# adrientremblay/Skillshot_Learning

Hardware: NVIDIA B200
Metric: env_steps_per_sec (higher is better)
Workload: dtype f64

## Files before the change

skillshot_learning_b200/csrc/ss_env.cu:

```cuda
#include <cuda_runtime.h>
#include <stdint.h>
#include <stdlib.h>

#include "../../include/skillshot_b200.h"
#include "ss_env_core.cuh"
#include "ss_env_pp.cuh"
#include "ss_launch.cuh"

namespace {

using namespace ss;

constexpr int kBlock = 64;
constexpr int kRowF4 = 7;

struct StatePlanes {
    double2 *rot;
    double2 *qrot;
    int4 *ia;
    int4 *ib;
};
__host__ __device__ inline StatePlanes planes_of(void *state, int64_t n) {
    char *b = (char *)state;
    return StatePlanes{(double2 *)b, (double2 *)(b + 16 * n), (int4 *)(b + 32 * n), (int4 *)(b + 48 * n)};
}

__device__ __forceinline__ void load_env(const StatePlanes &s, int64_t i, Env &e) {
    double2 r = s.rot[i], q = s.qrot[i];
    int4 a = s.ia[i], b = s.ib[i];
    unpack(e, r.x, r.y, q.x, q.y, Int4{a.x, a.y, a.z, a.w}, Int4{b.x, b.y, b.z, b.w});
}
__device__ __forceinline__ void store_env(const StatePlanes &s, int64_t i, const Env &e) {
    Int4 a, b;
    pack(e, a, b);
    s.rot[i] = make_double2(e.prot[0], e.prot[1]);
    s.qrot[i] = make_double2(e.qrot[0], e.qrot[1]);
    s.ia[i] = make_int4(a.x, a.y, a.z, a.w);
    s.ib[i] = make_int4(b.x, b.y, b.z, b.w);
}
__device__ __forceinline__ Speeds load_speeds(const void *speeds, int64_t n, int64_t i) {
    const char *b = (const char *)speeds;
    double2 a = ((const double2 *)b)[i];
    const double *p1 = (const double *)(b + 16 * n) + 2 * i;
    long long cm = ((const long long *)(b + 16 * n))[2 * i + 1];
    return Speeds{a.x, a.y, p1[0], (int)cm, 1.0f / (float)cm};
}

struct SmemSink {
    float4 *row;
    __device__ __forceinline__ void put(int j, float a, float b, float c, float d) { row[j] = make_float4(a, b, c, d); }
};

__device__ __noinline__ void count_episode(unsigned long long *stats, int len, int winner, int tick_limit) {
    const int width = tick_limit > 0 ? (tick_limit + 63) / 64 : 32;
    atomicAdd(stats + 0, 1ull);
    atomicAdd(stats + (winner == 1 ? 1 : winner == 2 ? 2 : 3), 1ull);
    atomicAdd(stats + 4, (unsigned long long)len);
    atomicAdd(stats + 8 + min(63, len / width), 1ull);
}

struct StepArgs {
    void *state;
    int64_t n;
    const float4 *actions;
    float4 *obs_out;
    float2 *reward_out;
    uint8_t *done_out;
    uint8_t *winner_out;
    float4 *obs_out2;
    uint16_t *done_rows_out;
    const void *speeds;
    uint32_t *status;
    unsigned long long *stats;
    uint8_t *packed_out;
    TickParams P;
    int n_ticks, obs_every_tick;
};

template <bool OBS, bool CARRY, bool SPEEDS, int MINB = 1, bool STATS = false, bool PDL = false, int BLK = kBlock>
__global__ void __launch_bounds__(BLK, MINB) step_kernel(const StepArgs A) {
    __shared__ float4 tile[OBS ? BLK / 32 : 1][OBS ? 32 * kRowF4 : 1];
    const int lane = threadIdx.x & 31, warp = threadIdx.x >> 5;
    const int64_t i = (int64_t)blockIdx.x * BLK + threadIdx.x;
    const int64_t warp_base = i - lane;
    const bool active = i < A.n;
    const StatePlanes S = planes_of(A.state, A.n);

    if (PDL) asm volatile("griddepcontrol.wait;" ::: "memory");
    Env e;
    Speeds k = default_speeds();
    if (active) {
        load_env(S, i, e);
        if (SPEEDS) k = load_speeds(A.speeds, A.n, i);
    } else {
        reset_env(e, 50, 50, 200, 200);
    }
    if (PDL) asm volatile("griddepcontrol.launch_dependents;");
    uint32_t status = 0;
    const bool write_reward = A.reward_out && A.P.reward_mode != SS_REWARD_NONE;
    Trig tr;
    if (CARRY) trig_of(e, tr);

    float4 a_next = make_float4(0.f, 0.f, 0.f, 0.f);
    if (active) a_next = __ldg(A.actions + i);
    for (int t = 0; t < A.n_ticks; ++t) {
        const int64_t row = (int64_t)t * A.n + i;
        const float4 a = a_next;
        if (active && t + 1 < A.n_ticks) a_next = __ldg(A.actions + row + A.n);
        const bool want_obs = OBS && (A.obs_every_tick || t == A.n_ticks - 1);
        float r[2];
        int done, winner;
        SmemSink sink{&tile[OBS ? warp : 0][OBS ? lane * kRowF4 : 0]};
        const int ticks_before = !STATS ? 0 : (!e.live || (A.P.tick_limit > 0 && e.ticks >= A.P.tick_limit)) ? -1 : e.ticks;
        tick_env<OBS, CARRY>(e, a.x, a.y, a.z, a.w, k, A.P, (uint64_t)i, t, want_obs, status, tr, r, done, winner, sink);
        if (STATS && active && done && ticks_before >= 0)
            count_episode(A.stats, ticks_before + 1, winner, (int)A.P.tick_limit);
        if (active) {
            if (write_reward) A.reward_out[row] = make_float2(r[0], r[1]);
            if (A.done_out) A.done_out[row] = (uint8_t)done;
            if (A.done_rows_out) A.done_rows_out[row] = (uint16_t)(winner ? 0x0101 : 0);
            if (A.winner_out) A.winner_out[row] = (uint8_t)winner;
        }
        if (OBS && want_obs) {
            __syncwarp();
            const int64_t tick_off = A.obs_every_tick ? (int64_t)t * A.n * 6 : 0;
            float4 *dst = A.obs_out + tick_off + warp_base * 6;
#pragma unroll
            for (int j = 0; j < 6; ++j) {
                int idx = j * 32 + lane, rw = idx / 6, cl = idx - rw * 6;
                if (warp_base + rw < A.n) {
                    const float4 v = tile[warp][rw * kRowF4 + cl];
                    dst[idx] = v;
                    if (A.obs_out2) A.obs_out2[warp_base * 6 + idx] = v;
                }
            }
            __syncwarp();
        }
    }
    if (active) store_env(S, i, e);
    if (status && A.status) atomicOr(A.status, status);
}

constexpr int kBlockPP = 64;
constexpr double kRound = 6755399441055744.0;

__device__ __forceinline__ double coord(int x) { return __hiloint2double(0x43380000, x); }
__device__ __forceinline__ int icoord(double w) { return __double2loint(w); }
__device__ __forceinline__ double with_low(double w, int lo) { return __hiloint2double(__double2hiint(w), lo); }

struct Lane {
    double rot;
    double s3, c3;
    double qs5, qc5;
    double wx, wy, ux, uy;
    int cd, age, valid, live, winner, ticks;
};

__device__ __forceinline__ float clip_unit_nan(float v) {
    float r;
    asm("max.NaN.f32 %0, %1, 0fBF800000;" : "=f"(r) : "f"(v));
    asm("min.NaN.f32 %0, %1, 0f3F800000;" : "=f"(r) : "f"(r));
    return r;
}
__device__ __forceinline__ bool either_nan(double a, double b) {
    int p;
    asm("{ .reg .pred q; setp.nan.f64 q, %1, %2; selp.s32 %0, 1, 0, q; }" : "=r"(p) : "d"(a), "d"(b));
    return p != 0;
}

__device__ __forceinline__ void lane_reset(Lane &L, double *qrot, int x, int y) {
    L.wx = coord(x); L.wy = coord(y); L.rot = 0.0;
    L.ux = coord(0); L.uy = coord(0); *qrot = 0.0; L.cd = 0; L.age = 0; L.valid = 0;
    L.ticks = 0; L.live = 1; L.winner = 0;
    L.s3 = 0.0; L.c3 = 3.0; L.qs5 = 0.0; L.qc5 = 5.0;
}

struct LaneIo {
    uint32_t idx;
    uint32_t n2;
    const float2 *actions;
    float *reward;
    uint8_t *flags;
};

struct Turn {
    double rot, s, c;
};

template <bool CHECKED>
__device__ __forceinline__ void turn_from(Turn &out, double rot_before, float look) {
    out.rot = fma((double)clip_unit_nan(look), 0.25, rot_before);
    if (CHECKED) sincos_d(out.rot, &out.s, &out.c);
    else sincos_d_unchecked(out.rot, &out.s, &out.c);
}

enum { OUT_FLAGS = 0, OUT_TERMINAL = 1, OUT_PACKED = 2 };

template <int TERMINAL, bool CHECKED>
__device__ __forceinline__ void lane_tick(Lane &L, double *qrot, const float move, const float look_next, const Turn &now, Turn &next,
                                          const StepArgs &A, LaneIo &io, int lane, int P, int64_t env, int tick, int limit,
                                          bool write_zero, bool &nan_seen) {
    turn_from<CHECKED>(next, now.rot, look_next);
    const double speed = (double)clip_unit_nan(move);
    const double vx = sub(sub(L.wx, kRound), mul(L.s3, speed));
    const double vy = sub(sub(L.wy, kRound), mul(L.c3, speed));
    const double cx = add(vx, kRound), cy = add(vy, kRound);
    const bool ok = (unsigned)icoord(cx) <= (unsigned)(kBoard - kPlayerSize) &&
                    (unsigned)icoord(cy) <= (unsigned)(kBoard - kPlayerSize);
    L.wx = with_low(L.wx, ok ? icoord(cx) : icoord(L.wx));
    L.wy = with_low(L.wy, ok ? icoord(cy) : icoord(L.wy));
    L.rot = now.rot;
    L.s3 = mul(now.s, 3.0); L.c3 = mul(now.c, 3.0);
    if (L.cd <= 0) {
        L.ux = with_low(L.ux, icoord(L.wx)); L.uy = with_low(L.uy, icoord(L.wy));
        *qrot = now.rot;
        L.qs5 = mul(now.s, 5.0); L.qc5 = mul(now.c, 5.0);
        L.valid = 1; L.cd = 15; L.age = 0;
    }
    const int lv = L.live;
    const double zx = sub(sub(L.ux, kRound), L.qs5);
    const double zy = sub(sub(L.uy, kRound), L.qc5);
    if (either_nan(vx, zx)) nan_seen = true;
    const double dx = add(zx, kRound), dy = add(zy, kRound);
    const bool inb = (unsigned)icoord(dx) <= (unsigned)(kBoard - kProjSize) &&
                     (unsigned)icoord(dy) <= (unsigned)(kBoard - kProjSize);
    const bool fly = lv && L.valid && inb;
    L.ux = with_low(L.ux, fly ? icoord(dx) : icoord(L.ux));
    L.uy = with_low(L.uy, fly ? icoord(dy) : icoord(L.uy));
    L.valid = lv ? (int)fly : L.valid;
    L.ticks += lv; L.cd -= lv; L.age += lv;
    const uint32_t mine = (uint32_t)icoord(L.ux) | ((uint32_t)icoord(L.uy) << 8) | ((uint32_t)L.valid << 16);
    const uint32_t theirs = __shfl_xor_sync(0xffffffffu, mine, 1);
    const int jx = theirs & 255, jy = (theirs >> 8) & 255, px = icoord(L.wx), py = icoord(L.wy);
    const bool in_x = (unsigned)(jx + kProjSize - px) <= (unsigned)kPlayerSize || (unsigned)(jx - px) <= (unsigned)kPlayerSize;
    const bool in_y = (unsigned)(jy - py) <= (unsigned)kPlayerSize || (unsigned)(jy - kProjSize - py) <= (unsigned)kPlayerSize;
    const bool hit = lv && (theirs >> 16) && in_x && in_y;
    const uint32_t pair = (__ballot_sync(0xffffffffu, hit) >> (lane & 30)) & 3u;
    float r = 0.f;
    if (pair) {
        L.winner = (pair & 1u) ? 1 : 2;
        L.live = 0;
        r = (L.winner - 1 == P) ? -1.f : 1.f;
    }
    const bool done = !L.live || L.ticks >= limit;
    if (TERMINAL == OUT_PACKED) {
        if (!P) io.flags[io.idx >> 1] = (uint8_t)((int)done | (L.winner << 1) | (pair ? 8 : 0));
    } else {
        if (TERMINAL == OUT_TERMINAL) io.reward[io.idx] = r;
        else if (write_zero) io.reward[io.idx] = 0.f;
        io.flags[io.idx >> 1] = (uint8_t)(P ? L.winner : (int)done);
    }
    io.idx += io.n2;
    if (A.P.auto_reset && done) {
        int x = P ? 200 : 50, y = x;
        if (A.P.reset_mode == SS_RESET_RANDOM) {
            const uint64_t ctr = A.P.counter + (uint64_t)tick;
            const U4 u = philox4x32_10(U4{(uint32_t)env, (uint32_t)((uint64_t)env >> 32), (uint32_t)ctr, (uint32_t)(ctr >> 32)},
                                       (uint32_t)A.P.seed, (uint32_t)(A.P.seed >> 32));
            x = rand_coord(P ? u.z : u.x); y = rand_coord(P ? u.w : u.y);
        }
        lane_reset(L, qrot, x, y);
        turn_from<CHECKED>(next, 0.0, look_next);
    }
}

template <int TERMINAL, bool CHECKED>
__device__ __forceinline__ void lane_loop(Lane &L, double *qrot, const StepArgs &A, LaneIo &io, int lane, int P, int64_t env,
                                          bool &nan_seen) {
    const int limit = A.P.tick_limit > 0 ? (int)min((int64_t)0x7fffffff, A.P.tick_limit) : 0x7fffffff;
    const bool write_zero = TERMINAL == OUT_FLAGS && A.reward_out && A.P.reward_mode != SS_REWARD_NONE;
    const int T = A.n_ticks;
    const float2 zero = make_float2(0.f, 0.f);
    float2 a0 = __ldg(io.actions + io.idx);
    float2 qa = T > 1 ? __ldg(io.actions + (io.idx + io.n2)) : zero;
    float2 qb = T > 2 ? __ldg(io.actions + (io.idx + 2 * io.n2)) : zero;
    Turn ta, tb;
    turn_from<CHECKED>(ta, L.rot, a0.y);
    float move = a0.x;
    for (int t = 0; t < T; t += 2) {
        lane_tick<TERMINAL, CHECKED>(L, qrot, move, qa.y, ta, tb, A, io, lane, P, env, t, limit, write_zero, nan_seen);
        move = qa.x;
        qa = (t + 3 < T) ? __ldg(io.actions + (io.idx + 2 * io.n2)) : zero;
        if (t + 1 < T) {
            lane_tick<TERMINAL, CHECKED>(L, qrot, move, qb.y, tb, ta, A, io, lane, P, env, t + 1, limit, write_zero, nan_seen);
            move = qb.x;
            qb = (t + 4 < T) ? __ldg(io.actions + (io.idx + 2 * io.n2)) : zero;
        }
    }
}

template <int TERMINAL, int BLK = kBlockPP>
__global__ void __launch_bounds__(BLK, 896 / BLK) step_pp_kernel(const StepArgs A) {
    constexpr int kBlockPP = BLK;
    __shared__ double qrot_sh[kBlockPP];
    const int lane = threadIdx.x & 31, P = lane & 1;
    int64_t gl = (int64_t)blockIdx.x * kBlockPP + threadIdx.x;
    gl = min(gl, 2 * A.n - 2 + P);
    const int64_t env = gl >> 1;
    char *const base = (char *)A.state;
    double *const qrot = &qrot_sh[threadIdx.x];
    Lane L;
    {
        L.rot = ((const double *)base)[gl];
        *qrot = ((const double *)(base + 16 * A.n))[gl];
        const int4 a = ((const int4 *)(base + 32 * A.n))[env], b = ((const int4 *)(base + 48 * A.n))[env];
        const uint32_t pp = (uint32_t)a.x >> (16 * P), qq = (uint32_t)a.y >> (16 * P), f = (uint32_t)b.w;
        L.wx = coord(pp & 255); L.wy = coord((pp >> 8) & 255); L.ux = coord(qq & 255); L.uy = coord((qq >> 8) & 255);
        L.cd = P ? a.w : a.z; L.age = P ? b.y : b.x; L.ticks = b.z;
        L.valid = (f >> P) & 1; L.live = (f >> 2) & 1; L.winner = (f >> 4) & 3;
        double s, c;
        sincos_d(L.rot, &s, &c);
        L.s3 = mul(s, 3.0); L.c3 = mul(c, 3.0);
        sincos_d(*qrot, &s, &c);
        L.qs5 = mul(s, 5.0); L.qc5 = mul(c, 5.0);
    }
    bool nan_seen = false;
    LaneIo io;
    io.idx = (uint32_t)gl; io.n2 = (uint32_t)(2 * A.n);
    io.actions = (const float2 *)A.actions;
    io.reward = (float *)A.reward_out;
    io.flags = TERMINAL == OUT_PACKED ? A.packed_out : (P ? A.winner_out : A.done_out);
    const bool in_range = fabs(L.rot) + 0.25 * (double)A.n_ticks + 1.0 < 1.0e5;
    if (__all_sync(0xffffffffu, in_range)) lane_loop<TERMINAL, false>(L, qrot, A, io, lane, P, env, nan_seen);
    else lane_loop<TERMINAL, true>(L, qrot, A, io, lane, P, env, nan_seen);
    const int v_other = __shfl_xor_sync(0xffffffffu, L.valid, 1);
    ((double *)base)[gl] = L.rot;
    ((double *)(base + 16 * A.n))[gl] = *qrot;
    char *ia = base + 32 * A.n + env * 16, *ib = base + 48 * A.n + env * 16;
    ((uint16_t *)ia)[P] = (uint16_t)(icoord(L.wx) | (icoord(L.wy) << 8));
    ((uint16_t *)ia)[2 + P] = (uint16_t)(icoord(L.ux) | (icoord(L.uy) << 8));
    ((int *)ia)[2 + P] = L.cd;
    ((int *)ib)[P] = L.age;
    if (!P) ((int2 *)ib)[1] = make_int2(L.ticks, L.valid | (v_other << 1) | (L.live << 2) | (L.winner << 4));
    if (nan_seen && A.status) atomicOr(A.status, kStatusNaN);
}

struct SelfPlayRows {
    static constexpr bool kPool = false;
};
struct PoolRows {
    static constexpr bool kPool = true;
    int64_t S, b;
    const float2 *opp_actions;
    float4 *opp_obs;
    unsigned long long *pool_stats;
};

__device__ __noinline__ void count_pool_game(unsigned long long *c, int len, int winner, int learner_player) {
    atomicAdd(c + 0, 1ull);
    atomicAdd(c + (winner == 0 ? 3 : winner == learner_player + 1 ? 2 : 1), 1ull);
    atomicAdd(c + 4, (unsigned long long)len);
}

template <bool STATS, class Rows>
__global__ void __launch_bounds__(kBlockPP) step_pp_obs_kernel(const StepArgs A, const Rows R) {
    __shared__ float4 tile[kBlockPP / 32][96];
    const int lane = threadIdx.x & 31, warp = threadIdx.x >> 5, P = lane & 1;
    const int64_t g0 = (int64_t)blockIdx.x * kBlockPP + threadIdx.x;
    const int64_t last = 2 * A.n - 2 + P;
    const bool active = g0 <= last;
    const int64_t gl = active ? g0 : last;
    const int64_t env = gl >> 1;
    sslaunch::griddep_wait();
    sslaunch::griddep_launch();
    bool learner = true;
    int64_t row = gl, block = 0;
    int learner_player = 0;
    if constexpr (Rows::kPool) {
        if (env >= R.S) {
            const int64_t j = env - R.S;
            block = j / R.b;
            learner_player = j - block * R.b >= (R.b >> 1) ? 1 : 0;
            learner = P == learner_player;
            row = learner ? 2 * R.S + j : j;
        }
    }
    sspp::LaneState L;
    sspp::lane_load((const char *)A.state, A.n, gl, L);
    const float2 *act = (const float2 *)A.actions;
    if constexpr (Rows::kPool) {
        if (!learner) act = R.opp_actions;
    }
    const float2 a = __ldg(act + row);
    uint32_t status = 0;
    sspp::LaneTrig T;
    sspp::lane_trig(L, T);
    sspp::LaneTickOut out;
    sspp::lane_obs_tick(L, T, a.x, a.y, A.P, (uint64_t)env, A.P.counter, lane, P, status, out);
    const int v_other = __shfl_xor_sync(0xffffffffu, L.valid, 1);
    if (active) {
        sspp::lane_store((char *)A.state, A.n, gl, L, v_other);
        if (learner && A.reward_out && A.P.reward_mode != SS_REWARD_NONE) ((float *)A.reward_out)[row] = out.reward;
        uint8_t *flag = P ? A.winner_out : A.done_out;
        if (flag) flag[env] = (uint8_t)(P ? out.winner : out.done);
        if (learner && A.done_rows_out) ((uint8_t *)A.done_rows_out)[row] = out.winner ? 1 : 0;
        if (STATS && !P && out.episode_len >= 0) count_episode(A.stats, out.episode_len, out.winner, (int)A.P.tick_limit);
        if constexpr (Rows::kPool) {
            if (!P && R.pool_stats && env >= R.S && out.episode_len >= 0)
                count_pool_game(R.pool_stats + block * 8, out.episode_len, out.winner, learner_player);
        }
    }
    if constexpr (Rows::kPool) {
        const unsigned lmask = __ballot_sync(0xffffffffu, active && learner), omask = __ballot_sync(0xffffffffu, active && !learner);
        const unsigned below = (1u << lane) - 1u;
        const int nl = __popc(lmask), no = __popc(omask);
        const int64_t l0 = __shfl_sync(0xffffffffu, row, lmask ? __ffs(lmask) - 1 : 0);
        const int64_t o0 = __shfl_sync(0xffffffffu, row, omask ? __ffs(omask) - 1 : 0);
        const int slot = learner ? __popc(lmask & below) : nl + __popc(omask & below);
        if (active) {
#pragma unroll
            for (int j = 0; j < 3; ++j) tile[warp][slot * 3 + j] = out.obs[j];
        }
        __syncwarp();
#pragma unroll
        for (int j = 0; j < 3; ++j) {
            const int idx = j * 32 + lane;
            if (idx < 3 * nl) {
                const float4 v = tile[warp][idx];
                A.obs_out[l0 * 3 + idx] = v;
                if (A.obs_out2) A.obs_out2[l0 * 3 + idx] = v;
            } else if (idx < 3 * (nl + no)) {
                R.opp_obs[o0 * 3 + (idx - 3 * nl)] = tile[warp][idx];
            }
        }
    } else {
#pragma unroll
        for (int j = 0; j < 3; ++j) tile[warp][lane * 3 + j] = out.obs[j];
        __syncwarp();
        const int64_t warp_base = (g0 - lane) * 3;
        const int64_t total = 2 * A.n * 3;
#pragma unroll
        for (int j = 0; j < 3; ++j) {
            const int64_t idx = warp_base + j * 32 + lane;
            if (idx < total) {
                const float4 v = tile[warp][j * 32 + lane];
                A.obs_out[idx] = v;
                if (A.obs_out2) A.obs_out2[idx] = v;
            }
        }
    }
    if (status && A.status) atomicOr(A.status, status);
}


struct TilesArgs {
    StepArgs S;
    int *tile_ready;
    int64_t units;
    int grid_fwd;
};

template <bool STATS>
__global__ void __launch_bounds__(32, 16) step_pp_tiles_kernel(const TilesArgs T) {
    const StepArgs &A = T.S;
    const int lane = threadIdx.x, P = lane & 1;
    const int per_step = 4 * T.grid_fwd;
    const int64_t j = blockIdx.x / per_step;
    const int c = (int)(blockIdx.x % per_step) >> 2, quarter = blockIdx.x & 3;
    const int64_t u0 = T.units * c / T.grid_fwd, u1 = T.units * (c + 1) / T.grid_fwd;
    const int64_t tile = u0 + j;
    if (tile >= u1) return;
    const int64_t rows = 2 * A.n;
    uint32_t status = 0;
    if (lane == 0) {
        int seen = 0;
        uint32_t spins = 0;
        for (;;) {
            asm volatile("ld.acquire.gpu.global.s32 %0, [%1];" : "=r"(seen) : "l"(T.tile_ready + tile) : "memory");
            if (seen >= 4) break;
            if (++spins > (1u << 20)) { status |= SS_STATUS_ROLLOUT_TIMEOUT; break; }
            __nanosleep(200);
        }
    }
    __syncwarp();
    const int64_t g0 = tile * 128 + quarter * 32 + lane;
    const int64_t last = rows - 2 + P;
    const bool active = g0 <= last;
    const int64_t gl = active ? g0 : last;
    const int64_t env = gl >> 1;
    sspp::LaneState L;
    sspp::lane_load((const char *)A.state, A.n, gl, L);
    const float2 a = __ldcg((const float2 *)A.actions + gl);
    sspp::LaneTrig Tr;
    sspp::lane_trig(L, Tr);
    sspp::LaneTickOut out;
    sspp::lane_obs_tick(L, Tr, a.x, a.y, A.P, (uint64_t)env, A.P.counter, lane, P, status, out);
    const int v_other = __shfl_xor_sync(0xffffffffu, L.valid, 1);
    if (active) {
        sspp::lane_store((char *)A.state, A.n, gl, L, v_other);
        if (A.reward_out && A.P.reward_mode != SS_REWARD_NONE) ((float *)A.reward_out)[gl] = out.reward;
        uint8_t *flag = P ? A.winner_out : A.done_out;
        if (flag) flag[env] = (uint8_t)(P ? out.winner : out.done);
        if (A.done_rows_out) ((uint8_t *)A.done_rows_out)[gl] = out.winner ? 1 : 0;
        if (STATS && !P && out.episode_len >= 0) sspp::count_episode_pp(A.stats, out.episode_len, out.winner, (int)A.P.tick_limit);
#pragma unroll
        for (int q = 0; q < 3; ++q) {
            A.obs_out[gl * 3 + q] = out.obs[q];
            if (A.obs_out2) A.obs_out2[gl * 3 + q] = out.obs[q];
        }
    }
    __syncwarp();
    if (lane == 0) atomicSub(T.tile_ready + tile, 1);
    if (status && A.status) atomicOr(A.status, status);
}

__global__ void reset_kernel(void *state, int64_t n, const uint8_t *mask, int reset_mode,
                             const int32_t *positions, uint64_t seed, uint64_t counter) {
    int64_t i = (int64_t)blockIdx.x * blockDim.x + threadIdx.x;
    if (i >= n) return;
    if (mask && !mask[i]) return;
    Env e;
    if (reset_mode == SS_RESET_GIVEN) {
        const int4 p = ((const int4 *)positions)[i];
        reset_env(e, p.x, p.y, p.z, p.w);
    } else if (reset_mode == SS_RESET_RANDOM) {
        reset_random(e, seed, (uint64_t)i, counter);
    } else {
        reset_env(e, 50, 50, 200, 200);
    }
    store_env(planes_of(state, n), i, e);
}

template <bool SPEEDS>
__global__ void features_kernel(const void *state, int64_t n, double *feat_out, double *obs_out,
                                int32_t *general_out, const void *speeds) {
    int64_t i = (int64_t)blockIdx.x * blockDim.x + threadIdx.x;
    if (i >= n) return;
    Env e;
    load_env(planes_of((void *)state, n), i, e);
    Speeds k = default_speeds();
    if (SPEEDS) k = load_speeds(speeds, n, i);
    if (general_out) {
        general_out[i * 3 + 0] = e.live; general_out[i * 3 + 1] = e.ticks; general_out[i * 3 + 2] = e.winner;
    }
    if (feat_out) {
        double f[kNumFeat];
        features_of<0>(e, f);
        for (int j = 0; j < kNumFeat; ++j) feat_out[(i * 2 + 0) * kNumFeat + j] = f[j];
        features_of<1>(e, f);
        for (int j = 0; j < kNumFeat; ++j) feat_out[(i * 2 + 1) * kNumFeat + j] = f[j];
    }
    if (obs_out) {
        double o[kNumObs];
        View v0 = view_of<0, false>(e), v1 = view_of<1, false>(e);
        obs_of<0>(e, v0, k, o);
        for (int j = 0; j < kNumObs; ++j) obs_out[(i * 2 + 0) * kNumObs + j] = o[j];
        obs_of<1>(e, v1, k, o);
        for (int j = 0; j < kNumObs; ++j) obs_out[(i * 2 + 1) * kNumObs + j] = o[j];
    }
}

__global__ void export_kernel(const void *state, int64_t n, int64_t first, int64_t count,
                              int32_t *ints, double *rots) {
    int64_t j = (int64_t)blockIdx.x * blockDim.x + threadIdx.x;
    if (j >= count) return;
    Env e;
    load_env(planes_of((void *)state, n), first + j, e);
    int32_t *o = ints + j * SS_EXPORT_INTS;
    o[0] = e.px[0]; o[1] = e.px[1]; o[2] = e.py[0]; o[3] = e.py[1];
    o[4] = e.qx[0]; o[5] = e.qx[1]; o[6] = e.qy[0]; o[7] = e.qy[1];
    o[8] = e.cd[0]; o[9] = e.cd[1]; o[10] = e.age[0]; o[11] = e.age[1];
    o[12] = e.valid[0]; o[13] = e.valid[1]; o[14] = e.ticks; o[15] = e.live; o[16] = e.winner;
    double *r = rots + j * 4;
    r[0] = e.prot[0]; r[1] = e.prot[1]; r[2] = e.qrot[0]; r[3] = e.qrot[1];
}

__global__ void import_kernel(void *state, int64_t n, int64_t first, int64_t count,
                              const int32_t *ints, const double *rots) {
    int64_t j = (int64_t)blockIdx.x * blockDim.x + threadIdx.x;
    if (j >= count) return;
    Env e;
    const int32_t *o = ints + j * SS_EXPORT_INTS;
    e.px[0] = o[0] & 255; e.px[1] = o[1] & 255; e.py[0] = o[2] & 255; e.py[1] = o[3] & 255;
    e.qx[0] = o[4] & 255; e.qx[1] = o[5] & 255; e.qy[0] = o[6] & 255; e.qy[1] = o[7] & 255;
    e.cd[0] = o[8]; e.cd[1] = o[9]; e.age[0] = o[10]; e.age[1] = o[11];
    e.valid[0] = o[12] != 0; e.valid[1] = o[13] != 0; e.ticks = o[14]; e.live = o[15] != 0; e.winner = o[16] & 3;
    const double *r = rots + j * 4;
    e.prot[0] = r[0]; e.prot[1] = r[1]; e.qrot[0] = r[2]; e.qrot[1] = r[3];
    store_env(planes_of(state, n), first + j, e);
}

template <int P>
__device__ void apply_player_op(Env &e, int op, double value, const Speeds &k, uint32_t &status) {
    double s, c;
    switch (op) {
        case SS_OP_MOVE_DIRECTION_FLOAT:
            sincos_d(e.prot[P], &s, &c);
            move_direction_float<P>(e, value, s, c, k, status);
            break;
        case SS_OP_MOVE_LOOK_FLOAT: move_look_float<P>(e, value, k); break;
        case SS_OP_SHOOT: move_shoot<P>(e, k); break;
        case SS_OP_MOVE_FORWARDS:
            sincos_d(e.prot[P], &s, &c);
            move_direction_float<P>(e, 1.0, s, c, k, status);
            break;
        case SS_OP_MOVE_BACKWARDS:
            sincos_d(e.prot[P], &s, &c);
            move_direction_float<P>(e, -1.0, s, c, k, status);
            break;
        case SS_OP_LOOK_LEFT: e.prot[P] = add(e.prot[P], k.speed_look); break;
        case SS_OP_LOOK_RIGHT: e.prot[P] = sub(e.prot[P], k.speed_look); break;
        default: break;
    }
}

__global__ void apply_kernel(void *state, int64_t n, int64_t env, int player, int op, double value,
                             const void *speeds, uint32_t *status_out) {
    Env e;
    const StatePlanes S = planes_of(state, n);
    load_env(S, env, e);
    Speeds k = speeds ? load_speeds(speeds, n, env) : default_speeds();
    uint32_t status = 0;
    if (op == SS_OP_GAME_TICK) {
        if (e.live) {
            double s, c;
            e.ticks += 1;
            sincos_d(e.qrot[0], &s, &c); proj_tick<0>(e, s, c, k, status);
            sincos_d(e.qrot[1], &s, &c); proj_tick<1>(e, s, c, k, status);
            check_collision(e);
        }
    } else if (player == 0) {
        apply_player_op<0>(e, op, value, k, status);
    } else {
        apply_player_op<1>(e, op, value, k, status);
    }
    store_env(S, env, e);
    if (status && status_out) atomicOr(status_out, status);
}

struct MatchStepArgs {
    void *state;
    int64_t n, split, tick_limit;
    const float2 *actions;
// ... 432 lines not shown
```

Before: 84.90 billion.

## Compute per-tick trig in f32 with exact f64 fallback near rounding boundaries

Replaces the per-tick f64 sincos and f64 position arithmetic with an f32 sincos and integer positions. Each rounded offset is checked against a safety margin and recomputed in f64 only when it lies near a .5 boundary. Projectile steps are precomputed once per spawn as integer offsets, so most ticks avoid f64 entirely. This is meant to cut FP64 throughput cost on the hot path, in exchange for extra branching, more code and a subtle exactness argument that relies on the margins.

```diff
diff --git a/skillshot_learning_b200/csrc/ss_env.cu b/skillshot_learning_b200/csrc/ss_env.cu
--- a/skillshot_learning_b200/csrc/ss_env.cu
+++ b/skillshot_learning_b200/csrc/ss_env.cu
@@ -5,6 +5,7 @@
 #include "../../include/skillshot_b200.h"
 #include "ss_env_core.cuh"
 #include "ss_env_pp.cuh"
+#include "ss_round_f32.cuh"
 #include "ss_launch.cuh"
 
 namespace {
@@ -156,6 +157,17 @@
     int cd, age, valid, live, winner, ticks;
 };
 
+struct LaneF {
+    double rot;
+    float s, c;
+    int px, py, ux, uy;
+    int sx, sy;
+    int qexact;
+    int cd, age, valid, live, winner, ticks;
+};
+
+struct ProjShared { double rot, s5, c5; };
+
 __device__ __forceinline__ float clip_unit_nan(float v) {
     float r;
     asm("max.NaN.f32 %0, %1, 0fBF800000;" : "=f"(r) : "f"(v));
@@ -167,12 +179,20 @@
     asm("{ .reg .pred q; setp.nan.f64 q, %1, %2; selp.s32 %0, 1, 0, q; }" : "=r"(p) : "d"(a), "d"(b));
     return p != 0;
 }
+__device__ __forceinline__ double i2d_exact(int x) { return sub(coord(x), kRound); }
+__device__ __forceinline__ int round_i(double v) { return icoord(add(v, kRound)); }
 
 __device__ __forceinline__ void lane_reset(Lane &L, double *qrot, int x, int y) {
     L.wx = coord(x); L.wy = coord(y); L.rot = 0.0;
     L.ux = coord(0); L.uy = coord(0); *qrot = 0.0; L.cd = 0; L.age = 0; L.valid = 0;
     L.ticks = 0; L.live = 1; L.winner = 0;
     L.s3 = 0.0; L.c3 = 3.0; L.qs5 = 0.0; L.qc5 = 5.0;
+}
+__device__ __forceinline__ void lane_reset(LaneF &L, ProjShared *q, int x, int y) {
+    L.px = x; L.py = y; L.rot = 0.0;
+    L.ux = 0; L.uy = 0; q->rot = 0.0; L.cd = 0; L.age = 0; L.valid = 0;
+    L.ticks = 0; L.live = 1; L.winner = 0;
+    L.s = 0.f; L.c = 1.f; L.sx = 0; L.sy = -5; L.qexact = 0;
 }
 
 struct LaneIo {
@@ -186,21 +206,74 @@
 struct Turn {
     double rot, s, c;
 };
-
-template <bool CHECKED>
+struct TurnF {
+    double rot;
+    float s, c;
+};
+
+__device__ __forceinline__ double turned(double rot_before, float look) {
+    return fma((double)clip_unit_nan(look), 0.25, rot_before);
+}
 __device__ __forceinline__ void turn_from(Turn &out, double rot_before, float look) {
-    out.rot = fma((double)clip_unit_nan(look), 0.25, rot_before);
-    if (CHECKED) sincos_d(out.rot, &out.s, &out.c);
-    else sincos_d_unchecked(out.rot, &out.s, &out.c);
+    out.rot = turned(rot_before, look);
+    sincos_d(out.rot, &out.s, &out.c);
+}
+__device__ __forceinline__ void turn_from(TurnF &out, double rot_before, float look) {
+    out.rot = turned(rot_before, look);
+    sincos_f32(out.rot, &out.s, &out.c);
 }
 
 enum { OUT_FLAGS = 0, OUT_TERMINAL = 1, OUT_PACKED = 2 };
 
-template <int TERMINAL, bool CHECKED>
+struct TickCtx {
+    const StepArgs &A;
+    LaneIo &io;
+    int lane, P;
+    int64_t env;
+    int limit;
+    bool write_zero;
+};
+
+template <int TERMINAL>
+__device__ __forceinline__ bool tick_end(const TickCtx &C, int px, int py, int ux, int uy, int valid, int lv, int &live, int &winner,
+                                         int ticks, int tick, int &x, int &y) {
+    const uint32_t mine = (uint32_t)ux | ((uint32_t)uy << 8) | ((uint32_t)valid << 16);
+    const uint32_t theirs = __shfl_xor_sync(0xffffffffu, mine, 1);
+    const int jx = theirs & 255, jy = (theirs >> 8) & 255;
+    const bool in_x = (unsigned)(jx + kProjSize - px) <= (unsigned)kPlayerSize || (unsigned)(jx - px) <= (unsigned)kPlayerSize;
+    const bool in_y = (unsigned)(jy - py) <= (unsigned)kPlayerSize || (unsigned)(jy - kProjSize - py) <= (unsigned)kPlayerSize;
+    const bool hit = lv && (theirs >> 16) && in_x && in_y;
+    const uint32_t pair = (__ballot_sync(0xffffffffu, hit) >> (C.lane & 30)) & 3u;
+    float r = 0.f;
+    if (pair) {
+        winner = (pair & 1u) ? 1 : 2;
+        live = 0;
+        r = (winner - 1 == C.P) ? -1.f : 1.f;
+    }
+    const bool done = !live || ticks >= C.limit;
+    if (TERMINAL == OUT_PACKED) {
+        if (!C.P) C.io.flags[C.io.idx >> 1] = (uint8_t)((int)done | (winner << 1) | (pair ? 8 : 0));
+    } else {
+        if (TERMINAL == OUT_TERMINAL) C.io.reward[C.io.idx] = r;
+        else if (C.write_zero) C.io.reward[C.io.idx] = 0.f;
+        C.io.flags[C.io.idx >> 1] = (uint8_t)(C.P ? winner : (int)done);
+    }
+    C.io.idx += C.io.n2;
+    if (!(C.A.P.auto_reset && done)) return false;
+    x = C.P ? 200 : 50; y = x;
+    if (C.A.P.reset_mode == SS_RESET_RANDOM) {
+        const uint64_t ctr = C.A.P.counter + (uint64_t)tick;
+        const U4 u = philox4x32_10(U4{(uint32_t)C.env, (uint32_t)((uint64_t)C.env >> 32), (uint32_t)ctr, (uint32_t)(ctr >> 32)},
+                                   (uint32_t)C.A.P.seed, (uint32_t)(C.A.P.seed >> 32));
+        x = rand_coord(C.P ? u.z : u.x); y = rand_coord(C.P ? u.w : u.y);
+    }
+    return true;
+}
+
+template <int TERMINAL>
 __device__ __forceinline__ void lane_tick(Lane &L, double *qrot, const float move, const float look_next, const Turn &now, Turn &next,
-                                          const StepArgs &A, LaneIo &io, int lane, int P, int64_t env, int tick, int limit,
-                                          bool write_zero, bool &nan_seen) {
-    turn_from<CHECKED>(next, now.rot, look_next);
+                                          const TickCtx &C, int tick, bool &nan_seen) {
+    turn_from(next, now.rot, look_next);
     const double speed = (double)clip_unit_nan(move);
     const double vx = sub(sub(L.wx, kRound), mul(L.s3, speed));
     const double vy = sub(sub(L.wy, kRound), mul(L.c3, speed));
@@ -229,60 +302,81 @@
     L.uy = with_low(L.uy, fly ? icoord(dy) : icoord(L.uy));
     L.valid = lv ? (int)fly : L.valid;
     L.ticks += lv; L.cd -= lv; L.age += lv;
-    const uint32_t mine = (uint32_t)icoord(L.ux) | ((uint32_t)icoord(L.uy) << 8) | ((uint32_t)L.valid << 16);
-    const uint32_t theirs = __shfl_xor_sync(0xffffffffu, mine, 1);
-    const int jx = theirs & 255, jy = (theirs >> 8) & 255, px = icoord(L.wx), py = icoord(L.wy);
-    const bool in_x = (unsigned)(jx + kProjSize - px) <= (unsigned)kPlayerSize || (unsigned)(jx - px) <= (unsigned)kPlayerSize;
-    const bool in_y = (unsigned)(jy - py) <= (unsigned)kPlayerSize || (unsigned)(jy - kProjSize - py) <= (unsigned)kPlayerSize;
-    const bool hit = lv && (theirs >> 16) && in_x && in_y;
-    const uint32_t pair = (__ballot_sync(0xffffffffu, hit) >> (lane & 30)) & 3u;
-    float r = 0.f;
-    if (pair) {
-        L.winner = (pair & 1u) ? 1 : 2;
-        L.live = 0;
-        r = (L.winner - 1 == P) ? -1.f : 1.f;
-    }
-    const bool done = !L.live || L.ticks >= limit;
-    if (TERMINAL == OUT_PACKED) {
-        if (!P) io.flags[io.idx >> 1] = (uint8_t)((int)done | (L.winner << 1) | (pair ? 8 : 0));
+    int x, y;
+    if (tick_end<TERMINAL>(C, icoord(L.wx), icoord(L.wy), icoord(L.ux), icoord(L.uy), L.valid, lv, L.live, L.winner, L.ticks, tick,
+                           x, y)) {
+        lane_reset(L, qrot, x, y);
+        turn_from(next, 0.0, look_next);
+    }
+}
+
+__device__ __forceinline__ void spawn_step(LaneF &L, ProjShared *q, double rot, float s, float c) {
+    L.qexact = proj_step(rot, s, c, &L.sx, &L.sy, &q->s5, &q->c5) == 2;
+}
+
+template <int TERMINAL>
+__device__ __forceinline__ void lane_tick(LaneF &L, ProjShared *q, const float move, const float look_next, const TurnF &now,
+                                          TurnF &next, const TickCtx &C, int tick, bool &nan_seen) {
+    turn_from(next, now.rot, look_next);
+    const float speed = clip_unit_nan(move);
+    int nx, ny;
+    if (move_offsets_f32(L.s, L.c, speed, &nx, &ny)) {
+        nx = L.px - nx; ny = L.py - ny;
     } else {
-        if (TERMINAL == OUT_TERMINAL) io.reward[io.idx] = r;
-        else if (write_zero) io.reward[io.idx] = 0.f;
-        io.flags[io.idx >> 1] = (uint8_t)(P ? L.winner : (int)done);
-    }
-    io.idx += io.n2;
-    if (A.P.auto_reset && done) {
-        int x = P ? 200 : 50, y = x;
-        if (A.P.reset_mode == SS_RESET_RANDOM) {
-            const uint64_t ctr = A.P.counter + (uint64_t)tick;
-            const U4 u = philox4x32_10(U4{(uint32_t)env, (uint32_t)((uint64_t)env >> 32), (uint32_t)ctr, (uint32_t)(ctr >> 32)},
-                                       (uint32_t)A.P.seed, (uint32_t)(A.P.seed >> 32));
-            x = rand_coord(P ? u.z : u.x); y = rand_coord(P ? u.w : u.y);
-        }
-        lane_reset(L, qrot, x, y);
-        turn_from<CHECKED>(next, 0.0, look_next);
-    }
-}
-
-template <int TERMINAL, bool CHECKED>
-__device__ __forceinline__ void lane_loop(Lane &L, double *qrot, const StepArgs &A, LaneIo &io, int lane, int P, int64_t env,
-                                          bool &nan_seen) {
-    const int limit = A.P.tick_limit > 0 ? (int)min((int64_t)0x7fffffff, A.P.tick_limit) : 0x7fffffff;
-    const bool write_zero = TERMINAL == OUT_FLAGS && A.reward_out && A.P.reward_mode != SS_REWARD_NONE;
-    const int T = A.n_ticks;
+        double s, c;
+        sincos_d_unchecked(L.rot, &s, &c);
+        const double sp = (double)speed;
+        const double vx = sub(i2d_exact(L.px), mul(mul(s, 3.0), sp));
+        const double vy = sub(i2d_exact(L.py), mul(mul(c, 3.0), sp));
+        if (either_nan(vx, vy)) nan_seen = true;
+        nx = round_i(vx); ny = round_i(vy);
+    }
+    if ((unsigned)nx <= (unsigned)(kBoard - kPlayerSize) && (unsigned)ny <= (unsigned)(kBoard - kPlayerSize)) {
+        L.px = nx; L.py = ny;
+    }
+    L.rot = now.rot; L.s = now.s; L.c = now.c;
+    if (L.cd <= 0) {
+        L.ux = L.px; L.uy = L.py;
+        q->rot = now.rot;
+        spawn_step(L, q, now.rot, now.s, now.c);
+        L.valid = 1; L.cd = 15; L.age = 0;
+    }
+    const int lv = L.live;
+    int mx = L.ux + L.sx, my = L.uy + L.sy;
+    if (L.qexact) {
+        const double zx = sub(i2d_exact(L.ux), q->s5), zy = sub(i2d_exact(L.uy), q->c5);
+        if (either_nan(zx, zy)) nan_seen = true;
+        mx = round_i(zx); my = round_i(zy);
+    }
+    const bool inb = (unsigned)mx <= (unsigned)(kBoard - kProjSize) && (unsigned)my <= (unsigned)(kBoard - kProjSize);
+    const bool fly = lv && L.valid && inb;
+    if (fly) { L.ux = mx; L.uy = my; }
+    L.valid = lv ? (int)fly : L.valid;
+    L.ticks += lv; L.cd -= lv; L.age += lv;
+    int x, y;
+    if (tick_end<TERMINAL>(C, L.px, L.py, L.ux, L.uy, L.valid, lv, L.live, L.winner, L.ticks, tick, x, y)) {
+        lane_reset(L, q, x, y);
+        turn_from(next, 0.0, look_next);
+    }
+}
+
+template <int TERMINAL, class LaneT, class TurnT, class Q>
+__device__ __forceinline__ void lane_loop(LaneT &L, Q *q, const TickCtx &C, bool &nan_seen) {
+    LaneIo &io = C.io;
+    const int T = C.A.n_ticks;
     const float2 zero = make_float2(0.f, 0.f);
     float2 a0 = __ldg(io.actions + io.idx);
     float2 qa = T > 1 ? __ldg(io.actions + (io.idx + io.n2)) : zero;
     float2 qb = T > 2 ? __ldg(io.actions + (io.idx + 2 * io.n2)) : zero;
-    Turn ta, tb;
-    turn_from<CHECKED>(ta, L.rot, a0.y);
+    TurnT ta, tb;
+    turn_from(ta, L.rot, a0.y);
     float move = a0.x;
     for (int t = 0; t < T; t += 2) {
-        lane_tick<TERMINAL, CHECKED>(L, qrot, move, qa.y, ta, tb, A, io, lane, P, env, t, limit, write_zero, nan_seen);
+        lane_tick<TERMINAL>(L, q, move, qa.y, ta, tb, C, t, nan_seen);
         move = qa.x;
         qa = (t + 3 < T) ? __ldg(io.actions + (io.idx + 2 * io.n2)) : zero;
         if (t + 1 < T) {
-            lane_tick<TERMINAL, CHECKED>(L, qrot, move, qb.y, tb, ta, A, io, lane, P, env, t + 1, limit, write_zero, nan_seen);
+            lane_tick<TERMINAL>(L, q, move, qb.y, tb, ta, C, t + 1, nan_seen);
             move = qb.x;
             qb = (t + 4 < T) ? __ldg(io.actions + (io.idx + 2 * io.n2)) : zero;
         }
@@ -292,27 +386,22 @@
 template <int TERMINAL, int BLK = kBlockPP>
 __global__ void __launch_bounds__(BLK, 896 / BLK) step_pp_kernel(const StepArgs A) {
     constexpr int kBlockPP = BLK;
-    __shared__ double qrot_sh[kBlockPP];
+    __shared__ ProjShared proj_sh[kBlockPP];
     const int lane = threadIdx.x & 31, P = lane & 1;
     int64_t gl = (int64_t)blockIdx.x * kBlockPP + threadIdx.x;
     gl = min(gl, 2 * A.n - 2 + P);
     const int64_t env = gl >> 1;
     char *const base = (char *)A.state;
-    double *const qrot = &qrot_sh[threadIdx.x];
-    Lane L;
+    ProjShared *const q = &proj_sh[threadIdx.x];
+    LaneF L;
     {
         L.rot = ((const double *)base)[gl];
-        *qrot = ((const double *)(base + 16 * A.n))[gl];
+        q->rot = ((const double *)(base + 16 * A.n))[gl];
         const int4 a = ((const int4 *)(base + 32 * A.n))[env], b = ((const int4 *)(base + 48 * A.n))[env];
         const uint32_t pp = (uint32_t)a.x >> (16 * P), qq = (uint32_t)a.y >> (16 * P), f = (uint32_t)b.w;
-        L.wx = coord(pp & 255); L.wy = coord((pp >> 8) & 255); L.ux = coord(qq & 255); L.uy = coord((qq >> 8) & 255);
+        L.px = pp & 255; L.py = (pp >> 8) & 255; L.ux = qq & 255; L.uy = (qq >> 8) & 255;
         L.cd = P ? a.w : a.z; L.age = P ? b.y : b.x; L.ticks = b.z;
         L.valid = (f >> P) & 1; L.live = (f >> 2) & 1; L.winner = (f >> 4) & 3;
-        double s, c;
-        sincos_d(L.rot, &s, &c);
-        L.s3 = mul(s, 3.0); L.c3 = mul(c, 3.0);
-        sincos_d(*qrot, &s, &c);
-        L.qs5 = mul(s, 5.0); L.qc5 = mul(c, 5.0);
     }
     bool nan_seen = false;
     LaneIo io;
@@ -320,15 +409,34 @@
     io.actions = (const float2 *)A.actions;
     io.reward = (float *)A.reward_out;
     io.flags = TERMINAL == OUT_PACKED ? A.packed_out : (P ? A.winner_out : A.done_out);
+    const TickCtx C{A, io, lane, P, env,
+                    A.P.tick_limit > 0 ? (int)min((int64_t)0x7fffffff, A.P.tick_limit) : 0x7fffffff,
+                    TERMINAL == OUT_FLAGS && A.reward_out && A.P.reward_mode != SS_REWARD_NONE};
     const bool in_range = fabs(L.rot) + 0.25 * (double)A.n_ticks + 1.0 < 1.0e5;
-    if (__all_sync(0xffffffffu, in_range)) lane_loop<TERMINAL, false>(L, qrot, A, io, lane, P, env, nan_seen);
-    else lane_loop<TERMINAL, true>(L, qrot, A, io, lane, P, env, nan_seen);
+    double s, c;
+    sincos_d(q->rot, &s, &c);
+    if (__all_sync(0xffffffffu, in_range)) {
+        sincos_f32(L.rot, &L.s, &L.c);
+        L.qexact = !proj_step_f64(s, c, &L.sx, &L.sy);
+        if (L.qexact) { q->s5 = mul(s, 5.0); q->c5 = mul(c, 5.0); }
+        lane_loop<TERMINAL, LaneF, TurnF>(L, q, C, nan_seen);
+    } else {
+        Lane D;
+        D.rot = L.rot; D.wx = coord(L.px); D.wy = coord(L.py); D.ux = coord(L.ux); D.uy = coord(L.uy);
+        D.cd = L.cd; D.age = L.age; D.valid = L.valid; D.live = L.live; D.winner = L.winner; D.ticks = L.ticks;
+        D.qs5 = mul(s, 5.0); D.qc5 = mul(c, 5.0);
+        sincos_d(D.rot, &s, &c);
+        D.s3 = mul(s, 3.0); D.c3 = mul(c, 3.0);
+        lane_loop<TERMINAL, Lane, Turn>(D, &q->rot, C, nan_seen);
+        L.rot = D.rot; L.px = icoord(D.wx); L.py = icoord(D.wy); L.ux = icoord(D.ux); L.uy = icoord(D.uy);
+        L.cd = D.cd; L.age = D.age; L.valid = D.valid; L.live = D.live; L.winner = D.winner; L.ticks = D.ticks;
+    }
     const int v_other = __shfl_xor_sync(0xffffffffu, L.valid, 1);
     ((double *)base)[gl] = L.rot;
-    ((double *)(base + 16 * A.n))[gl] = *qrot;
+    ((double *)(base + 16 * A.n))[gl] = q->rot;
     char *ia = base + 32 * A.n + env * 16, *ib = base + 48 * A.n + env * 16;
-    ((uint16_t *)ia)[P] = (uint16_t)(icoord(L.wx) | (icoord(L.wy) << 8));
-    ((uint16_t *)ia)[2 + P] = (uint16_t)(icoord(L.ux) | (icoord(L.uy) << 8));
+    ((uint16_t *)ia)[P] = (uint16_t)(L.px | (L.py << 8));
+    ((uint16_t *)ia)[2 + P] = (uint16_t)(L.ux | (L.uy << 8));
     ((int *)ia)[2 + P] = L.cd;
     ((int *)ib)[P] = L.age;
     if (!P) ((int2 *)ib)[1] = make_int2(L.ticks, L.valid | (v_other << 1) | (L.live << 2) | (L.winner << 4));
diff --git a/skillshot_learning_b200/csrc/ss_round_f32.cuh b/skillshot_learning_b200/csrc/ss_round_f32.cuh
--- /dev/null
+++ b/skillshot_learning_b200/csrc/ss_round_f32.cuh
@@ -0,0 +1,117 @@
+#pragma once
+#include "ss_env_core.cuh"
+
+namespace ss {
+
+SS_HD float fmul_rn(float a, float b) {
+#ifdef __CUDA_ARCH__
+    return __fmul_rn(a, b);
+#else
+    return a * b;
+#endif
+}
+SS_HD float fadd_rn(float a, float b) {
+#ifdef __CUDA_ARCH__
+    return __fadd_rn(a, b);
+#else
+    return a + b;
+#endif
+}
+SS_HD float ffma_rn(float a, float b, float c) {
+#ifdef __CUDA_ARCH__
+    return __fmaf_rn(a, b, c);
+#else
+    return fmaf(a, b, c);
+#endif
+}
+SS_HD float d2f_rn(double v) {
+#ifdef __CUDA_ARCH__
+    return __double2float_rn(v);
+#else
+    return (float)v;
+#endif
+}
+SS_HD int float_bits(float v) {
+#ifdef __CUDA_ARCH__
+    return __float_as_int(v);
+#else
+    int b; memcpy(&b, &v, sizeof b); return b;
+#endif
+}
+
+constexpr float kSinF1 = -1.6666654611e-1f, kSinF2 = 8.3321608736e-3f, kSinF3 = -1.9515295891e-4f;
+constexpr float kCosF1 = 4.166664568298827e-2f, kCosF2 = -1.388731625493765e-3f, kCosF3 = 2.443315711809948e-5f;
+
+SS_HD void sincos_f32_kernels(float t, float *sn, float *cs) {
+    const float z = fmul_rn(t, t);
+    float ps = ffma_rn(z, kSinF3, kSinF2);
+    ps = ffma_rn(ps, z, kSinF1);
+    *sn = ffma_rn(fmul_rn(t, z), ps, t);
+    float pc = ffma_rn(z, kCosF3, kCosF2);
+    pc = ffma_rn(pc, z, kCosF1);
+    *cs = ffma_rn(fmul_rn(z, z), pc, ffma_rn(-0.5f, z, 1.0f));
+}
+
+SS_HD void sincos_f32(double x, float *sp, float *cp) {
+    const double kMagic = SS_SC(0);
+    double q = fma(x, SS_SC(1), kMagic);
+    const int k = lo_word(q);
+    q = sub(q, kMagic);
+    double t = fma(q, SS_SC(2), x);
+    t = fma(q, SS_SC(3), t);
+    t = fma(q, SS_SC(4), t);
+    float sn, cs;
+    sincos_f32_kernels(d2f_rn(t), &sn, &cs);
+    const int swap = k & 1;
+    const float a = swap ? cs : sn, b = swap ? sn : cs;
+    *sp = ((k & 2) != 0) ? -a : a;
+    *cp = (((k + 1) & 2) != 0) ? -b : b;
+}
+
+constexpr float kEpsMove = 1.9073486328125e-6f;
+constexpr float kEpsProj = 3.814697265625e-6f;
+constexpr double kEpsProjExact = 5.684341886080802e-14;
+
+SS_HD bool round_clear_f32(float d, float eps, int *r) {
+    const float m = fadd_rn(d, 12582912.0f);
+    *r = float_bits(m) - 0x4B400000;
+    const float frac = fadd_rn(d, -fadd_rn(m, -12582912.0f));
+    return fabsf(frac) < 0.5f - eps;
+}
+SS_HD bool round_clear_f64(double d, double eps, int *r) {
+    const double m = add(d, 6755399441055744.0);
+    *r = lo_word(m);
+    return fabs(sub(d, sub(m, 6755399441055744.0))) < 0.5 - eps;
+}
+
+SS_HD bool move_offsets_f32(float s, float c, float speed, int *rx, int *ry) {
+    const bool ox = round_clear_f32(fmul_rn(fmul_rn(s, 3.0f), speed), kEpsMove, rx);
+    const bool oy = round_clear_f32(fmul_rn(fmul_rn(c, 3.0f), speed), kEpsMove, ry);
+    return ox && oy;
+}
+
+SS_HD bool proj_step_f32(float s, float c, int *sx, int *sy) {
+    int rx, ry;
+    const bool ox = round_clear_f32(fmul_rn(s, 5.0f), kEpsProj, &rx);
+    const bool oy = round_clear_f32(fmul_rn(c, 5.0f), kEpsProj, &ry);
+    *sx = -rx; *sy = -ry;
+    return ox && oy;
+}
+SS_HD bool proj_step_f64(double s, double c, int *sx, int *sy) {
+    int rx, ry;
+    const bool ox = round_clear_f64(mul(s, 5.0), kEpsProjExact, &rx);
+    const bool oy = round_clear_f64(mul(c, 5.0), kEpsProjExact, &ry);
+    *sx = -rx; *sy = -ry;
+    return ox && oy;
+}
+
+SS_HD int proj_step(double rot, float s, float c, int *sx, int *sy, double *s5, double *c5) {
+    if (proj_step_f32(s, c, sx, sy)) return 0;
+    double sd, cd;
+    sincos_d_unchecked(rot, &sd, &cd);
+    if (proj_step_f64(sd, cd, sx, sy)) return 1;
+    *s5 = mul(sd, 5.0); *c5 = mul(cd, 5.0);
+    return 2;
+}
+
+}
```

Result: faster. 92.35 billion, median of 6 (+8.8%).
